# mvenouziou/Boosted_DETR

Hardware: AMD Instinct MI355X
Metric: images/sec training step (fwd+matcher+loss+bwd), 640x640 N=100 (higher is better)
Workload: dtype f32 (conv/GEMM products as 3 split-f16 [fwd] / split-bf16 [grad] MFMA products, f32 accumulate)

## Files before the change

boosted_detr_amd/_lib.py:

```python
from __future__ import annotations

import ctypes as C
import os
from pathlib import Path

_LIB_PATH = Path(os.environ.get("BDETR_LIB") or Path(__file__).resolve().parent / "csrc" / "libbdetr.so")
_lib = None

c_f32p = C.c_void_p
c_i32p = C.c_void_p
c_i64p = C.c_void_p
c_stream = C.c_void_p


class ConvDesc(C.Structure):
    _fields_ = [(n, C.c_int) for n in ("N", "H", "W", "C", "K", "R", "S", "stride", "pad", "OH", "OW")]


class GemmDesc(C.Structure):
    _fields_ = [
        ("I", C.c_int), ("J", C.c_int), ("R", C.c_int), ("nb0", C.c_int), ("nb1", C.c_int),
        ("a", C.c_void_p), ("lda", C.c_int64), ("sa0", C.c_int64), ("sa1", C.c_int64), ("a_rcontig", C.c_int),
        ("b", C.c_void_p), ("ldb", C.c_int64), ("sb0", C.c_int64), ("sb1", C.c_int64), ("b_rcontig", C.c_int),
        ("c", C.c_void_p), ("ldc", C.c_int64), ("sc0", C.c_int64), ("sc1", C.c_int64),
# ... 42 lines not shown
SIGNATURES = {
    "bdetr_abi_version": (I, []),
    "bdetr_last_error": (C.c_char_p, []),
    "bdetr_device_cus": (I, []),
    "bdetr_low_priority_stream_create": (I, [P]),
    "bdetr_side_stream_candidates": (I, [P, I, I, I, P, P, P]),
    "bdetr_stream_destroy": (I, [P]),
    "bdetr_stream_priority_range": (I, [P, P]),
    "bdetr_set_gemm_precision": (I, [I]),
    "bdetr_get_gemm_precision": (I, []),
    "bdetr_prof_enable": (I, [I]),
    "bdetr_prof_read": (I, [P, P, P]),
    "bdetr_prof_read_arith": (I, [I, P, P, P]),
    "bdetr_prof_dump": (I, [C.c_char_p]),
    "bdetr_image_prep": (I, [P, I, I, I, P, I, I, P]),
    "bdetr_tokens_prepare": (I, [P, P, L, I, I, I, P, P, P]),
    "bdetr_augment_ws_floats": (I, [I]),
    "bdetr_augment": (I, [P, P, P, P, I, I, I, P, P]),
    "bdetr_jpeg_quality_ws_bytes": (C.c_int64, [I, I, I]),
    "bdetr_jpeg_quality": (I, [P, P, P, I, I, I, P, P]),
    "bdetr_augment_jpeg": (I, [P, P, P, P, P, I, I, I, P, P, P]),
    "bdetr_conv2d_fwd": (I, [P, P, P, P, C.POINTER(ConvDesc), I, P, P, P]),
    "bdetr_conv2d_fwd_stat_chunks": (I, [C.POINTER(ConvDesc)]),
    "bdetr_conv2d_bwd_data": (I, [P, P, P, C.POINTER(ConvDesc), I, P]),
    "bdetr_conv2d_bwd_weight": (I, [P, P, P, C.POINTER(ConvDesc), I, P]),
    "bdetr_conv2d_bwd_weight_splitk": (I, [C.POINTER(ConvDesc)]),
    "bdetr_bn_apply_p16": (I, [P, P, P, P, P, P, I, C.POINTER(BnAffine), I, P, P, P, P, P, L, I, P]),
    "bdetr_bn_apply_p16_even_pixels": (I, [P, P, P, P, P, P, I, C.POINTER(BnAffine), I, P, P, P, P, P, L, I, I, I, P]),
    "bdetr_bn_bwd_p16": (I, [P, P, I, P, P, P, P, P, I, I, P, P, P, P, P, P, P, P, I, L, I, P]),
    "bdetr_bn_bwd_p16_even_pixels": (I, [P, P, I, P, P, P, P, P, I, I, P, P, P, P, P, P, I, I, I, I, I, P]),
# ... 32 lines not shown
    "bdetr_bn_stats_fold_rows": (I, []),
    "bdetr_bn_stats_frozen": (I, [P, P, I, F, P, P, P]),
    "bdetr_bn_apply": (I, [P, P, P, P, P, P, I, P, L, I, P]),
    "bdetr_bn_bwd_chunks": (I, [L]),
    "bdetr_bn_bwd": (I, [P, P, P, P, P, P, P, I, I, P, P, P, P, P, L, I, P]),
    "bdetr_bn_rows_stats": (I, [P, I, L, I, F, P, P, P, P, P]),
    "bdetr_bn_rows_apply": (I, [P, P, P, P, P, P, I, L, I, I, P, F, P, P, P, P]),
    "bdetr_bn_rows_bwd": (I, [P, P, P, P, P, I, I, P, P, P, P, I, L, I, P]),
    "bdetr_maxpool3x3s2_fwd": (I, [P, P, I, I, I, I, I, I, P]),
    "bdetr_maxpool3x3s2_bwd": (I, [P, P, P, P, I, I, I, I, I, I, P]),
    "bdetr_stem_pool_bwd_chunks": (I, [L]),
    "bdetr_stem_pool_fwd": (I, [P, P, P, P, P, I, I, I, I, P, P, P, P, P]),
    "bdetr_stem_pool_bwd": (I, [P, P, P, P, P, P, P, I, I, I, I, P, I, P, P, P, P]),
    "bdetr_p16_s2d_pack_bf16": (I, [P, I, I, I, P, P]),
    "bdetr_p16_stem_bwd_weight": (I, [P, P, P, I, I, I, I, P]),
    "bdetr_p16_s2d_unpack_dw": (I, [P, P, I, P]),
    "bdetr_attention_head_dim": (I, []),
    "bdetr_attention_fwd": (I, [P, P, P, P, P, I, I, I, I, F, P]),
    "bdetr_attention_bwd": (I, [P, P, P, P, P, P, P, P, P, P, I, I, I, I, F, P]),
    "bdetr_softmax_rows_fwd": (I, [P, P, L, I, F, P]),
    "bdetr_softmax_rows_bwd": (I, [P, P, P, L, I, F, P]),
    "bdetr_add_dropout_layernorm_fwd": (I, [P, P, P, P, P, P, P, L, I, F, F, U64, P, P]),
    "bdetr_ln_bwd_chunks": (I, [L]),
    "bdetr_add_dropout_layernorm_bwd": (I, [P, P, P, P, P, P, P, P, P, P, P, L, I, F, U64, P, I, P]),
    "bdetr_rowchain_fwd": (I, [C.POINTER(RowchainFwdDesc), P]),
    "bdetr_rowchain_bwd": (I, [C.POINTER(RowchainBwdDesc), P]),
    "bdetr_rowchain_reduce": (I, [P, I, C.POINTER(C.c_void_p * 7), C.POINTER(C.c_int * 7), P]),
    "bdetr_rowchain_width": (I, []),
    "bdetr_rowchain_pack_elems": (L, []),
    "bdetr_rowchain_partial_rows": (I, [L]),
# ... 88 lines not shown
```

boosted_detr_amd/backbone.py:

```python
from __future__ import annotations

from . import kernels as K
from . import ops
from .engine import Layer

RESNET50_STAGES = ((64, 3, 1), (128, 4, 2), (256, 6, 2), (512, 3, 2))
RESNET101_STAGES = ((64, 3, 1), (128, 4, 2), (256, 23, 2), (512, 3, 2))
RESNET_BN_EPS = 1.001e-5
KERAS_BN_EPS = 1e-3


class _ConvBN(Layer):

    def __init__(self, prefix: str, conv_name: str, bn_name: str, cin: int, cout: int, ksize: int, stride: int, pad: int,
                 pad_in_channels: int = 0, **kw):
        super().__init__(name=conv_name, scope_prefix=prefix, **kw)
        self.stride, self.pad = stride, pad
        self.kernel = self.add_weight("kernel", (ksize, ksize, cin, cout), "glorot_uniform", kind="conv_kernel",
                                      pad_in_channels=pad_in_channels)
        self.bias = self.add_weight("bias", (cout,), "zeros")
        self.name = bn_name
        gamma = self.add_weight("gamma", (cout,), "ones")
        beta = self.add_weight("beta", (cout,), "zeros")
        mm = self.add_weight("moving_mean", (cout,), "zeros", trainable=False)
# ... 66 lines not shown
        self.ImageFeaturesExtractor = ResNet(stages, name="resnet50" if model_name != "ResNet101" else "resnet101",
                                             scope_prefix=f"{self.scope}/", **kwargs)
        self.built = True

    def config(self):
        return self.get_config()

    def get_config(self):
        c = super().get_config()
        c.update({"image_input_shape": self.image_input_shape})
        return c

    def call(self, inputs, training=False):
        image = inputs[0]
        height, width = self.image_input_shape[:2]
        x = ops.image_prep(image, height, width)
        return self.ImageFeaturesExtractor([x], training=training)


class BackboneNeck(Layer):

    def __init__(self, encoder_dim, name="BackboneNeck", **kwargs):
        super().__init__(name=name, **kwargs)
        self.encoder_dim = encoder_dim

    def get_config(self):
        c = super().get_config()
        c.update({"encoder_dim": self.encoder_dim})
        return c

    def _bn(self, bn_name, c):
# ... 25 lines not shown
```

boosted_detr_amd/csrc/elementwise.hip:

```cpp
#include "common.h"

namespace {

__device__ __forceinline__ float prep_px(float v) {
    float q = floorf(v * 255.5f);
    return fminf(fmaxf(q, 0.f), 255.f);
}

__global__ __launch_bounds__(256) void image_prep_kernel(const float* __restrict__ in, int B, int h, int w,
                                                         float* __restrict__ out, int H, int W) {
    const int64_t npix = (int64_t)B * H * W;
    const float sy = (float)h / (float)H, sx = (float)w / (float)W;
    for (int64_t i = (int64_t)blockIdx.x * blockDim.x + threadIdx.x; i < npix; i += (int64_t)gridDim.x * blockDim.x) {
        const int ox = (int)(i % W); const int64_t t = i / W; const int oy = (int)(t % H); const int b = (int)(t / H);
        float rgb[3];
        if (h == H && w == W) {
            const float* p = in + i * 3;
#pragma unroll
            for (int c = 0; c < 3; ++c) rgb[c] = fminf(fmaxf(p[c], 0.f), 1.f);
        } else {
            const float fy = ((float)oy + 0.5f) * sy - 0.5f, fx = ((float)ox + 0.5f) * sx - 0.5f;
            const float fy0 = floorf(fy), fx0 = floorf(fx);
            const int y0 = max((int)fy0, 0), y1 = min((int)ceilf(fy), h - 1);
            const int x0 = max((int)fx0, 0), x1 = min((int)ceilf(fx), w - 1);
            const float ly = fy - fy0, lx = fx - fx0;
            const float* base = in + (int64_t)b * h * w * 3;
#pragma unroll
            for (int c = 0; c < 3; ++c) {
                auto px = [&](int yy, int xx) { return fminf(fmaxf(base[((int64_t)yy * w + xx) * 3 + c], 0.f), 1.f); };
                const float top = px(y0, x0) + (px(y0, x1) - px(y0, x0)) * lx;
                const float bot = px(y1, x0) + (px(y1, x1) - px(y1, x0)) * lx;
                rgb[c] = top + (bot - top) * ly;
            }
        }
        f32x4 o;
        o[0] = prep_px(rgb[2]) - 103.939f;
        o[1] = prep_px(rgb[1]) - 116.779f;
        o[2] = prep_px(rgb[0]) - 123.68f;
        o[3] = 0.f;
        reinterpret_cast<f32x4*>(out)[i] = o;
    }
}

__global__ __launch_bounds__(256) void maxpool_fwd_kernel(const float* __restrict__ x, float* __restrict__ y,
                                                          int N, int H, int W, int C, int OH, int OW) {
    const int c4n = C / 4;
    const int64_t n4 = (int64_t)N * OH * OW * c4n;
    for (int64_t i = (int64_t)blockIdx.x * blockDim.x + threadIdx.x; i < n4; i += (int64_t)gridDim.x * blockDim.x) {
        const int c4 = (int)(i % c4n); int64_t t = i / c4n;
        const int ow = (int)(t % OW); t /= OW; const int oh = (int)(t % OH); const int n = (int)(t / OH);
        f32x4 m = {-INFINITY, -INFINITY, -INFINITY, -INFINITY};
#pragma unroll
        for (int r = 0; r < 3; ++r)
#pragma unroll
            for (int s = 0; s < 3; ++s) {
// ... 191 lines not shown
                       reinterpret_cast<unsigned long long*>(log), cursor, cap, (unsigned long long)tag);
    return bdetr_launch_status("debug_checksum");
}

extern "C" int bdetr_flag_nonfinite(const float* x, int64_t n, int* flag, void* stream) {
    BDETR_CHECK_ARG(x && flag && n > 0, "bdetr_flag_nonfinite: bad arguments");
    hipLaunchKernelGGL(flag_nonfinite_kernel, dim3(ew_grid(n, 256, 4)), dim3(256), 0, (hipStream_t)stream, x, n, flag);
    return bdetr_launch_status("flag_nonfinite");
}

extern "C" int bdetr_image_prep(const float* in, int B, int h, int w, float* out, int H, int W, void* stream) {
    BDETR_CHECK_ARG(in && out && B > 0 && h > 0 && w > 0 && H > 0 && W > 0, "bdetr_image_prep: bad arguments");
    int64_t n = (int64_t)B * H * W;
    hipLaunchKernelGGL(image_prep_kernel, dim3(ew_grid(n, 256, 1)), dim3(256), 0, (hipStream_t)stream, in, B, h, w, out, H, W);
    return bdetr_launch_status("image_prep");
}

extern "C" int bdetr_maxpool3x3s2_fwd(const float* x, float* y, int N, int H, int W, int C, int OH, int OW, void* stream) {
    BDETR_CHECK_ARG(x && y && C % 4 == 0 && OH == (H + 2 - 3) / 2 + 1 && OW == (W + 2 - 3) / 2 + 1, "bdetr_maxpool3x3s2_fwd: bad arguments");
    int64_t n4 = (int64_t)N * OH * OW * (C / 4);
    hipLaunchKernelGGL(maxpool_fwd_kernel, dim3(ew_grid(n4, 256, 1)), dim3(256), 0, (hipStream_t)stream, x, y, N, H, W, C, OH, OW);
    return bdetr_launch_status("maxpool_fwd");
}
extern "C" int bdetr_maxpool3x3s2_bwd(const float* x, const float* y, const float* dy, float* dx,
                                      int N, int H, int W, int C, int OH, int OW, void* stream) {
    BDETR_CHECK_ARG(x && y && dy && dx && C % 4 == 0 && OH == (H + 2 - 3) / 2 + 1 && OW == (W + 2 - 3) / 2 + 1, "bdetr_maxpool3x3s2_bwd: bad arguments");
    int64_t n4 = (int64_t)N * H * W * (C / 4);
    hipLaunchKernelGGL(maxpool_bwd_kernel, dim3(ew_grid(n4, 256, 1)), dim3(256), 0, (hipStream_t)stream, x, y, dy, dx, N, H, W, C, OH, OW);
    return bdetr_launch_status("maxpool_bwd");
}
// ... 165 lines not shown
```

boosted_detr_amd/csrc/p16.hip:

```cpp
#include "p16.h"

namespace {

__global__ __launch_bounds__(256) void p16_pack_kernel(const float* __restrict__ x, int64_t n8, void* __restrict__ f16_out, void* __restrict__ bf16_out,
                                                       int* __restrict__ overflow_flag, float f16_scale) {
    for (int64_t i = (int64_t)blockIdx.x * blockDim.x + threadIdx.x; i < n8; i += (int64_t)gridDim.x * blockDim.x) {
        const f32x4 a = reinterpret_cast<const f32x4*>(x)[2 * i], b = reinterpret_cast<const f32x4*>(x)[2 * i + 1];
        const float v[8] = {a[0], a[1], a[2], a[3], b[0], b[1], b[2], b[3]};
        if (f16_out) {
            const float vs[8] = {v[0] * f16_scale, v[1] * f16_scale, v[2] * f16_scale, v[3] * f16_scale, v[4] * f16_scale, v[5] * f16_scale, v[6] * f16_scale, v[7] * f16_scale};
            p16_store8<true>(reinterpret_cast<char*>(f16_out) + i * 32, vs);
            if (overflow_flag && p16_f16_overflow(vs)) *overflow_flag = 1;
        }
        if (bf16_out) p16_store8<false>(reinterpret_cast<char*>(bf16_out) + i * 32, v);
    }
}

template <bool F16>
__global__ __launch_bounds__(256) void p16_unpack_kernel(const void* __restrict__ p, int64_t n8, float* __restrict__ out) {
    for (int64_t i = (int64_t)blockIdx.x * blockDim.x + threadIdx.x; i < n8; i += (int64_t)gridDim.x * blockDim.x) {
        float v[8];
        p16_load8<F16>(reinterpret_cast<const char*>(p) + i * 32, v);
        reinterpret_cast<f32x4*>(out)[2 * i] = f32x4{v[0], v[1], v[2], v[3]};
        reinterpret_cast<f32x4*>(out)[2 * i + 1] = f32x4{v[4], v[5], v[6], v[7]};
// ... 30 lines not shown
            if (overflow_flag && p16_f16_overflow(v)) *overflow_flag = 1;
        }
        if (wt != nullptr) {
            const int c = (int)(i % C); int64_t t = i / C;
            const int tap = (int)(t % (R * S)); const int kg = (int)(t / (R * S));
            const int r = tap / S, s2 = tap - r * S;
            const int src_tap = (R - 1 - r) * S + (S - 1 - s2);
            float v[8];
#pragma unroll
            for (int e = 0; e < 8; ++e) v[e] = w[((int64_t)(kg * 8 + e) * R * S + src_tap) * C + c];
            p16_store8<false>(wt + (((int64_t)c * R * S + tap) * K + kg * 8) * 4, v);
        }
    }
}

}

extern "C" int bdetr_p16_pack_conv_weights_multi(const int64_t* table, int ntensors, int* overflow_flag, void* stream) {
    BDETR_CHECK_ARG(table && ntensors > 0, "bdetr_p16_pack_conv_weights_multi: bad arguments");
    hipLaunchKernelGGL(p16_pack_weights_multi_kernel, dim3(48, ntensors), dim3(256), 0, (hipStream_t)stream, table, overflow_flag);
    return bdetr_launch_status("p16_pack_conv_weights_multi");
}

extern "C" int bdetr_p16_pack(const float* x, int64_t n, void* f16_out, void* bf16_out, int* overflow_flag, void* stream) {
    BDETR_CHECK_ARG(x && n > 0 && n % 8 == 0 && (f16_out || bf16_out), "bdetr_p16_pack: bad arguments (n %% 8 == 0 required)");
    hipLaunchKernelGGL(p16_pack_kernel, dim3(ew_grid(n / 8, 256, 2)), dim3(256), 0, (hipStream_t)stream, x, n / 8, f16_out, bf16_out, overflow_flag, 1.f);
    return bdetr_launch_status("p16_pack");
}

extern "C" int bdetr_p16_unpack(const void* p, int is_f16, int64_t n, float* out, void* stream) {
    BDETR_CHECK_ARG(p && out && n > 0 && n % 8 == 0, "bdetr_p16_unpack: bad arguments (n %% 8 == 0 required)");
    if (is_f16) hipLaunchKernelGGL((p16_unpack_kernel<true>), dim3(ew_grid(n / 8, 256, 2)), dim3(256), 0, (hipStream_t)stream, p, n / 8, out);
    else        hipLaunchKernelGGL((p16_unpack_kernel<false>), dim3(ew_grid(n / 8, 256, 2)), dim3(256), 0, (hipStream_t)stream, p, n / 8, out);
    return bdetr_launch_status("p16_unpack");
}
// ... 46 lines not shown
```

boosted_detr_amd/csrc/sgemm.hip:

```cpp
#include "gemm_common.h"
#include "p16.h"
#include <stdlib.h>
#include <string.h>
#include <type_traits>
#include <utility>

using namespace bdgemm;

namespace {

constexpr int BK = 32;
constexpr unsigned OOB = 0xFFFFFFF0u;
constexpr unsigned NUM_RECORDS = 0xFFFFFF00u;

typedef __bf16 bf16x8 __attribute__((ext_vector_type(8)));
typedef _Float16 f16x8 __attribute__((ext_vector_type(8)));
typedef unsigned int u32x4 __attribute__((ext_vector_type(4)));
typedef unsigned int u32x2 __attribute__((ext_vector_type(2)));
typedef short s16x4 __attribute__((ext_vector_type(4)));
typedef __attribute__((address_space(3))) void lds_void;

__device__ __forceinline__ __amdgpu_buffer_rsrc_t make_rsrc(const void* p, unsigned records = NUM_RECORDS) {
    const unsigned long long a = reinterpret_cast<unsigned long long>(p);
    const unsigned lo = __builtin_amdgcn_readfirstlane((unsigned)a), hi = __builtin_amdgcn_readfirstlane((unsigned)(a >> 32));
// ... 958 lines not shown
    return splitk_fold(ws, zdim, slab, dw, n, st);
}
extern "C" int bdetr_p16_conv2d_bwd_weight_ws(const void* x, int x_is_f16, const void* dy_bf16, float* dw,
                                              const bdetr_conv_desc* d, int splitk, float* ws, int64_t ws_elems, void* stream) {
    return p16_bwd_weight(x, x_is_f16, dy_bf16, dw, d, splitk, stream, ws, ws_elems);
}
extern "C" int bdetr_p16_conv2d_bwd_weight(const void* x_bf16, const void* dy_bf16, float* dw,
                                           const bdetr_conv_desc* d, int splitk, void* stream) {
    return p16_bwd_weight(x_bf16, 0, dy_bf16, dw, d, splitk, stream);
}
extern "C" int bdetr_p16_conv2d_bwd_weight_xf16(const void* x_f16, const void* dy_bf16, float* dw,
                                                const bdetr_conv_desc* d, int splitk, void* stream) {
    return p16_bwd_weight(x_f16, 1, dy_bf16, dw, d, splitk, stream);
}

extern "C" int bdetr_p16_stem_bwd_weight(const void* x2_bf16, const void* dy_bf16, float* dw2, int N, int H2, int W2, int K, void* stream) {
    BDETR_CHECK_ARG(x2_bf16 && dy_bf16 && dw2 && N > 0 && H2 > 0 && W2 > 0 && K > 0 && K % 64 == 0 && aligned16(x2_bf16) && aligned16(dy_bf16),
                    "bdetr_p16_stem_bwd_weight: bad arguments (K %% 64 == 0)");
    const int64_t M64 = (int64_t)N * H2 * W2;
    BDETR_CHECK_ARG(M64 < (1LL << 31) && span_ok(M64 * 16) && span_ok(M64 * K), "bdetr_p16_stem_bwd_weight: tensors of 4 GB or more");
    const int M = (int)M64, Kd = 4 * 4 * 16;
    GemmParams g; init_params(g);
    g.I = K; g.J = Kd; g.R = M; g.c = dw2; g.ldc = Kd;
    const int64_t tiles = cdiv64(K, 64) * cdiv64(Kd, 64);
    int64_t sk = (16LL * num_cus()) / tiles;
    const int64_t maxsk = cdiv64(M, 8LL * BK);
    if (sk > maxsk) sk = maxsk;
    if (sk < 1) sk = 1;
    if (sk > 1024) sk = 1024;
    int zdim = 1;
    if (sk > 1) {
        g.r_chunk = (int)(cdiv64(cdiv64(M, sk), BK) * BK);
        zdim = (int)cdiv64(M, g.r_chunk);
        g.splitk = zdim > 1 ? zdim : 2;
        g.mode = ST_ATOMIC;
    }
    PDense a{dy_bf16, (unsigned)K, M, K};
    PPatch b = make_patch(x2_bf16, N, H2, W2, 16, H2, W2, 4, 4, 1, 2, M, Kd);
    return launch_any<XXDense, XXPatch, true, false>(a, b, g, zdim, (hipStream_t)stream, 3000, T_64x64);
}
```

boosted_detr_amd/kernels.py:

```python
from __future__ import annotations

import ctypes as C
from dataclasses import dataclass
from typing import Optional, Tuple

import numpy as np
import torch

from . import _lib
from ._lib import BnAffine, BnBwdFuse, ConvDesc, GemmDesc, LossDesc, RowchainBwdDesc, RowchainFwdDesc, check

ACT_NONE, ACT_RELU, ACT_TANH = 0, 1, 2


_LAUNCH_STREAM = [None]


def set_launch_stream(handle: Optional[int]) -> Optional[int]:
    prev = _LAUNCH_STREAM[0]
    _LAUNCH_STREAM[0] = handle
    return prev


GEMM_FP32, GEMM_BF16X3, GEMM_MIXED, GEMM_SPLIT, GEMM_BF16X6 = 0, 1, 2, 3, 4
# ... 77 lines not shown
        if not t.is_contiguous():
            raise _lib.BdetrError("kernel operands must be contiguous")


def empty(*shape, like: torch.Tensor, dtype=torch.float32) -> torch.Tensor:
    return torch.empty(shape, dtype=dtype, device=like.device)


def image_prep(image: torch.Tensor, H: int, W: int) -> torch.Tensor:
    _chk(image)
    B, h, w, c = image.shape
    assert c == 3
    out = empty(B, H, W, 4, like=image)
    check(_lib.lib().bdetr_image_prep(_p(image), B, h, w, _p(out), H, W, _stream()), "image_prep")
    return out


def tokens_prepare(cat_ids: torch.Tensor, att_ids: torch.Tensor, C_: int, A: int):
    _chk(cat_ids, att_ids, dtype=torch.int32)
    if cat_ids.dim() == 3:
        cat_ids = cat_ids[..., 0].contiguous()
    B, M = cat_ids.shape
    slots = att_ids.shape[2] if att_ids.dim() == 3 else 1
    cat = torch.empty_like(cat_ids)
    hot = torch.empty((B, M, A), dtype=torch.float32, device=cat_ids.device)
    check(_lib.lib().bdetr_tokens_prepare(_p(cat_ids), _p(att_ids), B * M, slots, C_, A, _p(cat), _p(hot), _stream()), "tokens_prepare")
    return cat, hot


def augment(image: torch.Tensor, iparams: torch.Tensor, fparams: torch.Tensor, quality: Optional[torch.Tensor] = None) -> torch.Tensor:
# ... 554 lines not shown

def stem_pool_bwd(dpool, tap, y, mean, rstd, gamma, beta, dgamma=None, dbeta=None, dy_p16=False):
    _chk(dpool, y, mean, rstd, gamma, beta, dgamma, dbeta)
    assert tap.is_cuda and tap.is_contiguous() and tap.dtype == torch.uint8 and tuple(tap.shape) == tuple(dpool.shape)
    L = _lib.lib()
    N, H, W, Cc = y.shape
    dy = torch.empty_like(y)
    dgamma = empty(Cc, like=y) if dgamma is None else dgamma
    dbeta = empty(Cc, like=y) if dbeta is None else dbeta
    ws = empty(2 * Cc * L.bdetr_stem_pool_bwd_chunks(N * H * W), like=y)
    check(L.bdetr_stem_pool_bwd(_p(dpool), _p(tap), _p(y), _p(mean), _p(rstd), _p(gamma), _p(beta), N, H, W, Cc, _p(dy), int(dy_p16), _p(dgamma), _p(dbeta),
                                _p(ws), _stream()), "stem_pool_bwd")
    return dy, dgamma, dbeta


def stem_bwd_weight_s2d(x4, dy_bf16, dw):
    _chk(x4, dy_bf16, dw)
    L = _lib.lib()
    N, H, W, Cc = x4.shape
    Kout = dw.shape[0]
    assert Cc == 4 and H % 2 == 0 and W % 2 == 0 and tuple(dw.shape) == (Kout, 7, 7, 4) and tuple(dy_bf16.shape) == (N, H // 2, W // 2, Kout)
    x2 = empty(N, H // 2, W // 2, 16, like=x4)
    check(L.bdetr_p16_s2d_pack_bf16(_p(x4), N, H, W, _p(x2), _stream()), "p16_s2d_pack_bf16")
    dw2 = empty(Kout, 4, 4, 16, like=x4)
    check(L.bdetr_zero(_p(dw2), dw2.numel(), _stream()), "zero")
    check(L.bdetr_p16_stem_bwd_weight(_p(x2), _p(dy_bf16), _p(dw2), N, H // 2, W // 2, Kout, _stream()), "p16_stem_bwd_weight")
    check(L.bdetr_p16_s2d_unpack_dw(_p(dw2), _p(dw), Kout, _stream()), "p16_s2d_unpack_dw")
    return dw


def attention_fwd(q, k, v, heads, scale):
    _chk(q, k, v)
    B, nq, D = q.shape
    nk = k.shape[1]
    o = empty(B, heads, nq, D // heads, like=q)
    lse = empty(B, heads, nq, like=q)
    check(_lib.lib().bdetr_attention_fwd(_p(q), _p(k), _p(v), _p(o), _p(lse), B, heads, nq, nk, scale, _stream()), "attention_fwd")
    return o, lse


def attention_bwd(q, k, v, o, d_o, lse, heads, scale):
# ... 809 lines not shown
```

boosted_detr_amd/ops.py:

```python
from __future__ import annotations

import math
import os
import weakref
from typing import Optional

import numpy as np
import torch

from . import kernels as K
from . import _lib
from .engine import WEIGHTS_VERSION, Variable, capture, current_tape, dense_contribution, info, materialise, own, side_task, tag

_dropout_site = [0]
_dropout_seed_dev = [None]


def dropout_seed_tensor() -> torch.Tensor:
    if _dropout_seed_dev[0] is None:
        _dropout_seed_dev[0] = torch.full((1,), 0x5EED, dtype=torch.int64, device="cuda")
    return _dropout_seed_dev[0]


def set_dropout_seed(seed: int, write: bool = True) -> None:
# ... 476 lines not shown
        g, mine = g.contiguous(), info(g).owned
        return tuple(own(g[l * B:(l + 1) * B]) if mine else g[l * B:(l + 1) * B] for l in range(L))

    _rec([out], list(xs), backward)
    return out


def maxpool(x: torch.Tensor) -> torch.Tensor:
    y = K.maxpool_fwd(x)
    _rec([y], [x], lambda g: (own(K.maxpool_bwd(x, y, g.contiguous())),))
    return y


STEM_FUSE = os.environ.get("BDETR_STEM_FUSE", "1") != "0"
STEM_S2D = os.environ.get("BDETR_STEM_S2D", "1") != "0"


def conv_bn_relu_maxpool(x: torch.Tensor, w: Variable, b: Variable, bn: BNState, stride: int, pad: int, training: bool,
                         bn_batch_stats: bool) -> torch.Tensor:
    N, H, W, Cin = x.shape
    Kout, R, S, _ = w.value.shape
    if not (STEM_FUSE and training and bn_batch_stats and _p16_active() and Kout % 8 == 0):
        return maxpool(conv_bn(x, w, b, bn, stride, pad, True, training=training, bn_batch_stats=bn_batch_stats, x_needs_grad=False))
    g = K.ConvGeom(N, H, W, Cin, Kout, R, S, stride, pad)
    x32 = as_fp32(x)
    y, parts = K.conv2d_fwd(x32, w.value, b.value, g, K.ACT_NONE, want_stats=True)
    if parts is None or parts[0] is None:
        parts = K.colstats(_2d(y))
    mean, rstd = K.bn_stats(g.M, Kout, parts, bn.eps, bn.momentum, True, bn.moving_mean.value, bn.moving_var.value, like=y)
    _, out, tap = K.stem_pool_fwd(y, mean, rstd, bn.gamma.value, bn.beta.value)
    attach_packed(out, out.detach(), p16_only=True)

    def backward(g_out):
        sg, sb = GradSink(bn.gamma), GradSink(bn.beta)
        s2d = (STEM_S2D and w.needs_grad and (R, S, stride, pad, Cin) == (7, 7, 2, 3, 4) and H % 2 == 0 and W % 2 == 0 and Kout % 64 == 0
               and K.get_gemm_precision() in ("split", "mixed") and not K.deterministic())
        dy, _, _ = K.stem_pool_bwd(materialise(g_out).contiguous(), tap, y, mean, rstd, bn.gamma.value, bn.beta.value, dgamma=sg.buf, dbeta=sb.buf,
                                   dy_p16=s2d)
        sg.commit()
        sb.commit()
        if s2d:
            _param_grads_task(w, b, lambda dw, pz: K.stem_bwd_weight_s2d(x32, dy, dw), None, x32, dy)
        else:
            _param_grads_task(w, b, lambda dw, pz: K.conv2d_bwd_weight(x32, dy, g, dw=dw, prezeroed=pz), None, x32, dy)
        return (None,)

    _rec([out], [x], backward)
    return out


def dense(x: torch.Tensor, w: Variable, b: Variable, act: int = K.ACT_NONE) -> torch.Tensor:
    x2d = _2d(x)
    y2d = K.linear_fwd(x2d, w.value, b.value, act)
    y = y2d.view(*x.shape[:-1], w.value.shape[0])

    def backward(g_out, acc=None):
        g2d = _2d(g_out.contiguous())
# ... 279 lines not shown
```

boosted_detr_amd/training.py:

```python
from __future__ import annotations

import contextlib
import glob
import math
import os
import sys
import time
from dataclasses import dataclass
from typing import Dict, Iterable, List, NamedTuple, Optional

import numpy as np
import torch

from . import _lib
from . import engine
from . import kernels as K
from . import ops
from .inference import Inference
from .engine import Layer, Tape, Variable, bump_weights_version, device, join_side_stream, recording, to_device


class CosineDecayRestarts:

    def __init__(self, initial_learning_rate, first_decay_steps, t_mul=2.0, m_mul=1.0, alpha=0.0):
# ... 914 lines not shown
        entry = self._graphs.get(sig)
        if entry is None:
            n = self._graph_warm.get(sig, 0)
            self._graph_warm[sig] = n + 1
            if n < 2 or getattr(self.optimizer, "flat_grad", None) is None:
                return None
            static = {k: v.clone() for k, v in data.items()}
            ops.set_dropout_seed(self._step_seed())
            self.optimizer.stage_lr()
            keep = (self.steps_done, self.optimizer.iterations)
            if self._dp is not None:
                self._dp.drain()
            cap = engine.SegmentedCapture()
            engine.set_capture(cap)
            prev_launch = K.set_launch_stream(None)
            try:
                cap.begin_main()
                logs = self._device_step(static, stage_scalars=False)
                cap.end_main()
                cap.sides.append(None)
            except BaseException:
                cap.abort()
                self.steps_done, self.optimizer.iterations = keep
                raise
            finally:
                engine.set_capture(None)
                K.set_launch_stream(prev_launch)
            cap.done = []
            if cap.CENSUS:
                self._graph_census = cap.census()
            self.steps_done, self.optimizer.iterations = keep
            entry = (cap, static, logs, (list(self._step_losses), list(self._loss_roots), dict(self._step_metrics)))
            self._graphs[sig] = entry
        cap, static, logs, book = entry
        for k, v in data.items():
            if v is not static[k]:
                static[k].copy_(v)
        ops.set_dropout_seed(self._step_seed())
        self.optimizer.stage_lr()
        cap.replay(engine.side_stream() if os.environ.get("BDETR_GRAPH_SIDE", "1") != "0" else None)
# ... 152 lines not shown
```

include/bdetr.h:

```cpp
#ifndef BDETR_H
#define BDETR_H
#include <stdint.h>
#ifdef __cplusplus
extern "C" {
#endif

#define BDETR_ABI_VERSION 8

int         bdetr_abi_version(void);
const char* bdetr_last_error(void);
int         bdetr_device_cus(void);

int         bdetr_low_priority_stream_create(void** stream_out);
int         bdetr_stream_priority_range(int* least, int* greatest);
int         bdetr_side_stream_candidates(void* main_stream, int ncand, int loads, int ticks, void** streams_out, float* scores_ms, float* unloaded_ms);
int         bdetr_stream_destroy(void* stream);

enum { BDETR_GEMM_FP32 = 0, BDETR_GEMM_BF16X3 = 1, BDETR_GEMM_MIXED = 2, BDETR_GEMM_SPLIT = 3, BDETR_GEMM_BF16X6 = 4 };
int         bdetr_set_gemm_precision(int mode);
int         bdetr_get_gemm_precision(void);

int bdetr_prof_enable(int on);
int bdetr_prof_read(double* total_ms, int64_t* launches, double* flops);
int bdetr_prof_read_arith(int arith, double* total_ms, int64_t* launches, double* flops);
int bdetr_prof_dump(const char* path);

enum { BDETR_ACT_NONE = 0, BDETR_ACT_RELU = 1, BDETR_ACT_TANH = 2 };

int bdetr_image_prep(const float* in, int B, int h, int w, float* out, int H, int W, void* stream);

int bdetr_tokens_prepare(const int* cat_ids, const int* att_ids, int64_t rows, int slots, int C, int A,
                         int* cat_out, float* att_hot, void* stream);

int bdetr_augment_ws_floats(int B);
int bdetr_augment(const float* in, float* out, const int32_t* iparams, const float* fparams,
                  int B, int H, int W, float* ws, void* stream);
int64_t bdetr_jpeg_quality_ws_bytes(int B, int H, int W);
int bdetr_jpeg_quality(const float* in, float* out, const int32_t* quality, int B, int H, int W, void* ws, void* stream);
int bdetr_augment_jpeg(const float* in, float* out, const int32_t* iparams, const float* fparams, const int32_t* quality,
                       int B, int H, int W, float* ws, void* jpeg_ws, void* stream);

typedef struct {
    int N, H, W, C;
    int K, R, S;
// ... 111 lines not shown
int bdetr_bn_rows_bwd(const float* dout, const float* x, const float* mean, const float* rstd, const float* gamma,
                      int grouped_stats, int frozen, float* dx, float* dgamma, float* dbeta, float* ws, int G, int64_t R, int C,
                      void* stream);

int bdetr_maxpool3x3s2_fwd(const float* x, float* y, int N, int H, int W, int C, int OH, int OW, void* stream);
int bdetr_maxpool3x3s2_bwd(const float* x, const float* y, const float* dy, float* dx,
                           int N, int H, int W, int C, int OH, int OW, void* stream);

int bdetr_stem_pool_bwd_chunks(int64_t rows);
int bdetr_stem_pool_fwd(const float* y, const float* mean, const float* rstd, const float* gamma, const float* beta,
                        int N, int H, int W, int C, float* out32, void* out_f16, uint8_t* tap, int* overflow_flag, void* stream);
int bdetr_stem_pool_bwd(const float* dpool, const uint8_t* tap, const float* y, const float* mean, const float* rstd, const float* gamma,
                        const float* beta, int N, int H, int W, int C, float* dy, int dy_p16 , float* dgamma, float* dbeta, float* ws, void* stream);
int bdetr_p16_s2d_pack_bf16(const float* x, int N, int H, int W, void* out_bf16, void* stream);
int bdetr_p16_stem_bwd_weight(const void* x2_bf16, const void* dy_bf16, float* dw2, int N, int H2, int W2, int K, void* stream);
int bdetr_p16_s2d_unpack_dw(const float* dw2, float* dw, int K, void* stream);

int bdetr_softmax_rows_fwd(const float* s, float* p, int64_t rows, int cols, float scale, void* stream);
int bdetr_softmax_rows_bwd(const float* p, const float* dp, float* ds, int64_t rows, int cols, float scale, void* stream);

int bdetr_attention_head_dim(void);
int bdetr_attention_fwd(const float* q, const float* k, const float* v, float* o, float* lse,
                        int B, int h, int nq, int nk, float scale, void* stream);
int bdetr_attention_bwd(const float* q, const float* k, const float* v, const float* o, const float* d_o,
                        const float* lse, float* dq, float* dk, float* dv, float* dvec_ws,
                        int B, int h, int nq, int nk, float scale, void* stream);

int bdetr_add_dropout_layernorm_fwd(const float* x, const float* y, const float* gamma, const float* beta,
                                    float* out, float* mean, float* rstd, int64_t rows, int D,
                                    float eps, float rate, uint64_t seed, const uint64_t* seed_base, void* stream);
// ... 168 lines not shown
```

Baseline: 658.0.

## Fuse stem s2d packing into image prep, widen stem dW tile, tile weight packing

Image preprocessing now also writes the space-to-depth bf16 copy used by the stem weight-gradient GEMM, which removes a separate pack pass over the input. The dW2 buffer is zeroed during the forward pass instead of in backward. The stem bwd-weight GEMM uses a wider 64x256 tile with less split-K. A new tiled, LDS-transposed multi-tensor conv weight packing kernel replaces the old one, and Python GC is disabled during graph capture. The changes are mostly independent and add env switches plus extra code paths.

```diff
diff --git a/boosted_detr_amd/_lib.py b/boosted_detr_amd/_lib.py
--- a/boosted_detr_amd/_lib.py
+++ b/boosted_detr_amd/_lib.py
@@ -80,6 +80,7 @@
     "bdetr_prof_read_arith": (I, [I, P, P, P]),
     "bdetr_prof_dump": (I, [C.c_char_p]),
     "bdetr_image_prep": (I, [P, I, I, I, P, I, I, P]),
+    "bdetr_image_prep_s2d": (I, [P, I, I, I, P, I, I, P, P]),
     "bdetr_tokens_prepare": (I, [P, P, L, I, I, I, P, P, P]),
     "bdetr_augment_ws_floats": (I, [I]),
     "bdetr_augment": (I, [P, P, P, P, I, I, I, P, P]),
@@ -142,6 +143,7 @@
     "bdetr_stem_pool_bwd": (I, [P, P, P, P, P, P, P, I, I, I, I, P, I, P, P, P, P]),
     "bdetr_p16_s2d_pack_bf16": (I, [P, I, I, I, P, P]),
     "bdetr_p16_stem_bwd_weight": (I, [P, P, P, I, I, I, I, P]),
+    "bdetr_p16_stem_bwd_weight_splitk": (I, [P, P, P, I, I, I, I, I, P]),
     "bdetr_p16_s2d_unpack_dw": (I, [P, P, I, P]),
     "bdetr_attention_head_dim": (I, []),
     "bdetr_attention_fwd": (I, [P, P, P, P, P, I, I, I, I, F, P]),
diff --git a/boosted_detr_amd/backbone.py b/boosted_detr_amd/backbone.py
--- a/boosted_detr_amd/backbone.py
+++ b/boosted_detr_amd/backbone.py
@@ -104,7 +104,8 @@
     def call(self, inputs, training=False):
         image = inputs[0]
         height, width = self.image_input_shape[:2]
-        x = ops.image_prep(image, height, width)
+        st = self.ImageFeaturesExtractor.stem
+        x = ops.image_prep_for_stem(image, height, width, st.kernel, st.stride, st.pad, training, training and st.trainable)
         return self.ImageFeaturesExtractor([x], training=training)
 
 
diff --git a/boosted_detr_amd/csrc/elementwise.hip b/boosted_detr_amd/csrc/elementwise.hip
--- a/boosted_detr_amd/csrc/elementwise.hip
+++ b/boosted_detr_amd/csrc/elementwise.hip
@@ -1,10 +1,39 @@
-#include "common.h"
+#include "p16.h"
 
 namespace {
 
 __device__ __forceinline__ float prep_px(float v) {
     float q = floorf(v * 255.5f);
     return fminf(fmaxf(q, 0.f), 255.f);
+}
+
+__device__ __forceinline__ f32x4 image_prep_pixel(const float* __restrict__ in, int h, int w, int H, int W, float sy, float sx, int64_t i, int b, int oy, int ox) {
+    float rgb[3];
+    if (h == H && w == W) {
+        const float* p = in + i * 3;
+#pragma unroll
+        for (int c = 0; c < 3; ++c) rgb[c] = fminf(fmaxf(p[c], 0.f), 1.f);
+    } else {
+        const float fy = ((float)oy + 0.5f) * sy - 0.5f, fx = ((float)ox + 0.5f) * sx - 0.5f;
+        const float fy0 = floorf(fy), fx0 = floorf(fx);
+        const int y0 = max((int)fy0, 0), y1 = min((int)ceilf(fy), h - 1);
+        const int x0 = max((int)fx0, 0), x1 = min((int)ceilf(fx), w - 1);
+        const float ly = fy - fy0, lx = fx - fx0;
+        const float* base = in + (int64_t)b * h * w * 3;
+#pragma unroll
+        for (int c = 0; c < 3; ++c) {
+            auto px = [&](int yy, int xx) { return fminf(fmaxf(base[((int64_t)yy * w + xx) * 3 + c], 0.f), 1.f); };
+            const float top = px(y0, x0) + (px(y0, x1) - px(y0, x0)) * lx;
+            const float bot = px(y1, x0) + (px(y1, x1) - px(y1, x0)) * lx;
+            rgb[c] = top + (bot - top) * ly;
+        }
+    }
+    f32x4 o;
+    o[0] = prep_px(rgb[2]) - 103.939f;
+    o[1] = prep_px(rgb[1]) - 116.779f;
+    o[2] = prep_px(rgb[0]) - 123.68f;
+    o[3] = 0.f;
+    return o;
 }
 
 __global__ __launch_bounds__(256) void image_prep_kernel(const float* __restrict__ in, int B, int h, int w,
@@ -13,32 +42,23 @@
     const float sy = (float)h / (float)H, sx = (float)w / (float)W;
     for (int64_t i = (int64_t)blockIdx.x * blockDim.x + threadIdx.x; i < npix; i += (int64_t)gridDim.x * blockDim.x) {
         const int ox = (int)(i % W); const int64_t t = i / W; const int oy = (int)(t % H); const int b = (int)(t / H);
-        float rgb[3];
-        if (h == H && w == W) {
-            const float* p = in + i * 3;
-#pragma unroll
-            for (int c = 0; c < 3; ++c) rgb[c] = fminf(fmaxf(p[c], 0.f), 1.f);
-        } else {
-            const float fy = ((float)oy + 0.5f) * sy - 0.5f, fx = ((float)ox + 0.5f) * sx - 0.5f;
-            const float fy0 = floorf(fy), fx0 = floorf(fx);
-            const int y0 = max((int)fy0, 0), y1 = min((int)ceilf(fy), h - 1);
-            const int x0 = max((int)fx0, 0), x1 = min((int)ceilf(fx), w - 1);
-            const float ly = fy - fy0, lx = fx - fx0;
-            const float* base = in + (int64_t)b * h * w * 3;
-#pragma unroll
-            for (int c = 0; c < 3; ++c) {
-                auto px = [&](int yy, int xx) { return fminf(fmaxf(base[((int64_t)yy * w + xx) * 3 + c], 0.f), 1.f); };
-                const float top = px(y0, x0) + (px(y0, x1) - px(y0, x0)) * lx;
-                const float bot = px(y1, x0) + (px(y1, x1) - px(y1, x0)) * lx;
-                rgb[c] = top + (bot - top) * ly;
-            }
-        }
-        f32x4 o;
-        o[0] = prep_px(rgb[2]) - 103.939f;
-        o[1] = prep_px(rgb[1]) - 116.779f;
-        o[2] = prep_px(rgb[0]) - 123.68f;
-        o[3] = 0.f;
-        reinterpret_cast<f32x4*>(out)[i] = o;
+        reinterpret_cast<f32x4*>(out)[i] = image_prep_pixel(in, h, w, H, W, sy, sx, i, b, oy, ox);
+    }
+}
+
+__global__ __launch_bounds__(256) void image_prep_s2d_kernel(const float* __restrict__ in, int B, int h, int w,
+                                                             float* __restrict__ out, int H, int W, void* __restrict__ x2) {
+    const int H2 = H >> 1, W2 = W >> 1;
+    const int64_t n = (int64_t)B * H * W;
+    const float sy = (float)h / (float)H, sx = (float)w / (float)W;
+    for (int64_t u = (int64_t)blockIdx.x * blockDim.x + threadIdx.x; u < n; u += (int64_t)gridDim.x * blockDim.x) {
+        const int ab = (int)(u & 3); const int64_t t = u >> 2;
+        const int j = (int)(t % W2); const int64_t q = t / W2; const int i2 = (int)(q % H2); const int b = (int)(q / H2);
+        const int oy = 2 * i2 + (ab >> 1), ox = 2 * j + (ab & 1);
+        const int64_t i = ((int64_t)b * H + oy) * W + ox;
+        const f32x4 p = image_prep_pixel(in, h, w, H, W, sy, sx, i, b, oy, ox);
+        reinterpret_cast<f32x4*>(out)[i] = p;
+        p16_store4<false>(x2, u, p[0], p[1], p[2], p[3]);
     }
 }
 
@@ -260,6 +280,12 @@
     int64_t n = (int64_t)B * H * W;
     hipLaunchKernelGGL(image_prep_kernel, dim3(ew_grid(n, 256, 1)), dim3(256), 0, (hipStream_t)stream, in, B, h, w, out, H, W);
     return bdetr_launch_status("image_prep");
+}
+extern "C" int bdetr_image_prep_s2d(const float* in, int B, int h, int w, float* out, int H, int W, void* x2_bf16, void* stream) {
+    BDETR_CHECK_ARG(in && out && x2_bf16 && B > 0 && h > 0 && w > 0 && H > 0 && W > 0 && H % 2 == 0 && W % 2 == 0, "bdetr_image_prep_s2d: bad arguments (even H and W)");
+    int64_t n = (int64_t)B * H * W;
+    hipLaunchKernelGGL(image_prep_s2d_kernel, dim3(ew_grid(n, 256, 1)), dim3(256), 0, (hipStream_t)stream, in, B, h, w, out, H, W, x2_bf16);
+    return bdetr_launch_status("image_prep_s2d");
 }
 
 extern "C" int bdetr_maxpool3x3s2_fwd(const float* x, float* y, int N, int H, int W, int C, int OH, int OW, void* stream) {
diff --git a/boosted_detr_amd/csrc/p16.hip b/boosted_detr_amd/csrc/p16.hip
--- a/boosted_detr_amd/csrc/p16.hip
+++ b/boosted_detr_amd/csrc/p16.hip
@@ -1,4 +1,6 @@
 #include "p16.h"
+#include <stdlib.h>
+#include <string.h>
 
 namespace {
 
@@ -68,11 +70,93 @@
     }
 }
 
+constexpr int PACK_T = 64, PACK_LD = PACK_T + 1;
+constexpr int PACK_ROWS = 256;
+__global__ __launch_bounds__(256) void p16_pack_weights_tiled_kernel(const int64_t* __restrict__ table, int ntensors, int* __restrict__ overflow_flag) {
+    __shared__ float tile[PACK_T * PACK_LD];
+    __shared__ int last[PACK_ROWS];
+    const int tid = threadIdx.x;
+    {
+        int n = 0;
+        if (tid < ntensors) {
+            const int64_t* row = table + (int64_t)tid * 7;
+            if (row[1] != 0 || row[2] != 0) n = (int)(row[4] * row[5] * ((row[3] + PACK_T - 1) / PACK_T) * ((row[6] + PACK_T - 1) / PACK_T));
+        }
+        last[tid] = n;
+        __syncthreads();
+        for (int d = 1; d < PACK_ROWS; d <<= 1) {
+            const int v = tid >= d ? last[tid - d] : 0;
+            __syncthreads();
+            last[tid] += v;
+            __syncthreads();
+        }
+    }
+    const int total = last[PACK_ROWS - 1];
+    for (int item = blockIdx.x; item < total; item += gridDim.x) {
+        int t = 0;
+        for (int hi = ntensors - 1; t < hi;) { const int mid = (t + hi) >> 1; if (last[mid] > item) hi = mid; else t = mid + 1; }
+        const int64_t* row = table + (int64_t)t * 7;
+        const float* w = reinterpret_cast<const float*>(row[0]);
+        char* wf = reinterpret_cast<char*>(row[1]);
+        char* wt = reinterpret_cast<char*>(row[2]);
+        const int K = (int)row[3], T = (int)(row[4] * row[5]), C = (int)row[6];
+        const int ctiles = (C + PACK_T - 1) / PACK_T;
+        int q = item - (t > 0 ? last[t - 1] : 0);
+        const int c0 = (q % ctiles) * PACK_T; q /= ctiles;
+        const int src_tap = q % T, k0 = (q / T) * PACK_T;
+        const int g8 = tid & 7, r32 = tid >> 3;
+#pragma unroll
+        for (int pass = 0; pass < PACK_T / 32; ++pass) {
+            const int kl = pass * 32 + r32, k = k0 + kl, c = c0 + g8 * 8;
+            if (k < K && c < C) {
+                const int64_t at = ((int64_t)k * T + src_tap) * C + c;
+                const f32x4 a = *reinterpret_cast<const f32x4*>(w + at), b = *reinterpret_cast<const f32x4*>(w + at + 4);
+                if (wf != nullptr) {
+                    const float v[8] = {a[0] * P16_W_SCALE, a[1] * P16_W_SCALE, a[2] * P16_W_SCALE, a[3] * P16_W_SCALE,
+                                        b[0] * P16_W_SCALE, b[1] * P16_W_SCALE, b[2] * P16_W_SCALE, b[3] * P16_W_SCALE};
+                    p16_store8<true>(wf + at * 4, v);
+                    if (overflow_flag && p16_f16_overflow(v)) *overflow_flag = 1;
+                }
+                if (wt != nullptr) {
+                    float* d = tile + kl * PACK_LD + g8 * 8;
+                    d[0] = a[0]; d[1] = a[1]; d[2] = a[2]; d[3] = a[3]; d[4] = b[0]; d[5] = b[1]; d[6] = b[2]; d[7] = b[3];
+                }
+            }
+        }
+        if (wt != nullptr) {
+            __syncthreads();
+            const int tap = T - 1 - src_tap;
+#pragma unroll
+            for (int pass = 0; pass < PACK_T / 32; ++pass) {
+                const int cl = pass * 32 + r32, c = c0 + cl, k = k0 + g8 * 8;
+                if (c < C && k < K) {
+                    float v[8];
+#pragma unroll
+                    for (int e = 0; e < 8; ++e) v[e] = tile[(g8 * 8 + e) * PACK_LD + cl];
+                    p16_store8<false>(wt + (((int64_t)c * T + tap) * K + k) * 4, v);
+                }
+            }
+            __syncthreads();
+        }
+    }
+}
+
+bool pack_tiled() {
+    const char* e = getenv("BDETR_PACK_TILED");
+    return !(e && !strcmp(e, "0"));
+}
+
 }
 
 extern "C" int bdetr_p16_pack_conv_weights_multi(const int64_t* table, int ntensors, int* overflow_flag, void* stream) {
     BDETR_CHECK_ARG(table && ntensors > 0, "bdetr_p16_pack_conv_weights_multi: bad arguments");
-    hipLaunchKernelGGL(p16_pack_weights_multi_kernel, dim3(48, ntensors), dim3(256), 0, (hipStream_t)stream, table, overflow_flag);
+    if (pack_tiled()) {
+        for (int first = 0; first < ntensors; first += PACK_ROWS)
+            hipLaunchKernelGGL(p16_pack_weights_tiled_kernel, dim3(2048), dim3(256), 0, (hipStream_t)stream, table + (int64_t)first * 7,
+                               ntensors - first < PACK_ROWS ? ntensors - first : PACK_ROWS, overflow_flag);
+    } else {
+        hipLaunchKernelGGL(p16_pack_weights_multi_kernel, dim3(48, ntensors), dim3(256), 0, (hipStream_t)stream, table, overflow_flag);
+    }
     return bdetr_launch_status("p16_pack_conv_weights_multi");
 }
 
diff --git a/boosted_detr_amd/csrc/sgemm.hip b/boosted_detr_amd/csrc/sgemm.hip
--- a/boosted_detr_amd/csrc/sgemm.hip
+++ b/boosted_detr_amd/csrc/sgemm.hip
@@ -996,18 +996,23 @@
     return p16_bwd_weight(x_f16, 1, dy_bf16, dw, d, splitk, stream);
 }
 
-extern "C" int bdetr_p16_stem_bwd_weight(const void* x2_bf16, const void* dy_bf16, float* dw2, int N, int H2, int W2, int K, void* stream) {
+static int stem_wide_tile() {
+    const char* e = getenv("BDETR_STEM_DW_WIDE");
+    return (e && !strcmp(e, "0")) ? 0 : 1;
+}
+extern "C" int bdetr_p16_stem_bwd_weight_splitk(const void* x2_bf16, const void* dy_bf16, float* dw2, int N, int H2, int W2, int K, int splitk, void* stream) {
     BDETR_CHECK_ARG(x2_bf16 && dy_bf16 && dw2 && N > 0 && H2 > 0 && W2 > 0 && K > 0 && K % 64 == 0 && aligned16(x2_bf16) && aligned16(dy_bf16),
                     "bdetr_p16_stem_bwd_weight: bad arguments (K %% 64 == 0)");
     const int64_t M64 = (int64_t)N * H2 * W2;
     BDETR_CHECK_ARG(M64 < (1LL << 31) && span_ok(M64 * 16) && span_ok(M64 * K), "bdetr_p16_stem_bwd_weight: tensors of 4 GB or more");
     const int M = (int)M64, Kd = 4 * 4 * 16;
+    const bool wide = stem_wide_tile() != 0;
     GemmParams g; init_params(g);
     g.I = K; g.J = Kd; g.R = M; g.c = dw2; g.ldc = Kd;
-    const int64_t tiles = cdiv64(K, 64) * cdiv64(Kd, 64);
-    int64_t sk = (16LL * num_cus()) / tiles;
+    const int64_t tiles = cdiv64(K, 64) * cdiv64(Kd, wide ? 256 : 64);
+    int64_t sk = splitk > 0 ? splitk : ((wide ? 2LL : 16LL) * num_cus()) / tiles;
     const int64_t maxsk = cdiv64(M, 8LL * BK);
-    if (sk > maxsk) sk = maxsk;
+    if (splitk <= 0 && sk > maxsk) sk = maxsk;
     if (sk < 1) sk = 1;
     if (sk > 1024) sk = 1024;
     int zdim = 1;
@@ -1019,5 +1024,9 @@
     }
     PDense a{dy_bf16, (unsigned)K, M, K};
     PPatch b = make_patch(x2_bf16, N, H2, W2, 16, H2, W2, 4, 4, 1, 2, M, Kd);
+    if (wide) return launch_cfg<64, 256, 2, 4, 2, XXDense, XXPatch, true, false, false, 4>(a, b, g, zdim, (hipStream_t)stream, 3000);
     return launch_any<XXDense, XXPatch, true, false>(a, b, g, zdim, (hipStream_t)stream, 3000, T_64x64);
 }
+extern "C" int bdetr_p16_stem_bwd_weight(const void* x2_bf16, const void* dy_bf16, float* dw2, int N, int H2, int W2, int K, void* stream) {
+    return bdetr_p16_stem_bwd_weight_splitk(x2_bf16, dy_bf16, dw2, N, H2, W2, K, 0, stream);
+}
diff --git a/boosted_detr_amd/kernels.py b/boosted_detr_amd/kernels.py
--- a/boosted_detr_amd/kernels.py
+++ b/boosted_detr_amd/kernels.py
@@ -115,6 +115,22 @@
     out = empty(B, H, W, 4, like=image)
     check(_lib.lib().bdetr_image_prep(_p(image), B, h, w, _p(out), H, W, _stream()), "image_prep")
     return out
+
+
+def image_prep_s2d(image: torch.Tensor, H: int, W: int):
+    _chk(image)
+    B, h, w, c = image.shape
+    assert c == 3 and H % 2 == 0 and W % 2 == 0
+    out = empty(B, H, W, 4, like=image)
+    x2 = empty(B, H // 2, W // 2, 16, like=image)
+    check(_lib.lib().bdetr_image_prep_s2d(_p(image), B, h, w, _p(out), H, W, _p(x2), _stream()), "image_prep_s2d")
+    return out, x2
+
+
+def stem_dw2_zeros(Kout: int, like: torch.Tensor) -> torch.Tensor:
+    dw2 = empty(Kout, 4, 4, 16, like=like)
+    check(_lib.lib().bdetr_zero(_p(dw2), dw2.numel(), _stream()), "zero")
+    return dw2
 
 
 def tokens_prepare(cat_ids: torch.Tensor, att_ids: torch.Tensor, C_: int, A: int):
@@ -699,17 +715,19 @@
     return dy, dgamma, dbeta
 
 
-def stem_bwd_weight_s2d(x4, dy_bf16, dw):
-    _chk(x4, dy_bf16, dw)
+def stem_bwd_weight_s2d(x4, dy_bf16, dw, splitk: int = 0, x2=None, dw2=None):
+    _chk(x4, dy_bf16, dw, x2, dw2)
     L = _lib.lib()
     N, H, W, Cc = x4.shape
     Kout = dw.shape[0]
     assert Cc == 4 and H % 2 == 0 and W % 2 == 0 and tuple(dw.shape) == (Kout, 7, 7, 4) and tuple(dy_bf16.shape) == (N, H // 2, W // 2, Kout)
-    x2 = empty(N, H // 2, W // 2, 16, like=x4)
-    check(L.bdetr_p16_s2d_pack_bf16(_p(x4), N, H, W, _p(x2), _stream()), "p16_s2d_pack_bf16")
-    dw2 = empty(Kout, 4, 4, 16, like=x4)
-    check(L.bdetr_zero(_p(dw2), dw2.numel(), _stream()), "zero")
-    check(L.bdetr_p16_stem_bwd_weight(_p(x2), _p(dy_bf16), _p(dw2), N, H // 2, W // 2, Kout, _stream()), "p16_stem_bwd_weight")
+    if x2 is None:
+        x2 = empty(N, H // 2, W // 2, 16, like=x4)
+        check(L.bdetr_p16_s2d_pack_bf16(_p(x4), N, H, W, _p(x2), _stream()), "p16_s2d_pack_bf16")
+    if dw2 is None:
+        dw2 = stem_dw2_zeros(Kout, x4)
+    assert tuple(x2.shape) == (N, H // 2, W // 2, 16) and tuple(dw2.shape) == (Kout, 4, 4, 16)
+    check(L.bdetr_p16_stem_bwd_weight_splitk(_p(x2), _p(dy_bf16), _p(dw2), N, H // 2, W // 2, Kout, int(splitk), _stream()), "p16_stem_bwd_weight")
     check(L.bdetr_p16_s2d_unpack_dw(_p(dw2), _p(dw), Kout, _stream()), "p16_s2d_unpack_dw")
     return dw
 
diff --git a/boosted_detr_amd/ops.py b/boosted_detr_amd/ops.py
--- a/boosted_detr_amd/ops.py
+++ b/boosted_detr_amd/ops.py
@@ -514,13 +514,35 @@
 
 STEM_FUSE = os.environ.get("BDETR_STEM_FUSE", "1") != "0"
 STEM_S2D = os.environ.get("BDETR_STEM_S2D", "1") != "0"
+STEM_S2D_PREP = os.environ.get("BDETR_STEM_S2D_PREP", "1") != "0"
+
+
+def _stem_s2d(x_shape, w: Variable, stride: int, pad: int) -> bool:
+    _, H, W, Cin = x_shape
+    Kout, R, S, _ = w.value.shape
+    return (STEM_S2D and w.needs_grad and (R, S, stride, pad, Cin) == (7, 7, 2, 3, 4) and H % 2 == 0 and W % 2 == 0 and Kout % 64 == 0
+            and K.get_gemm_precision() in ("split", "mixed") and not K.deterministic())
+
+
+def _stem_fused(w: Variable, training: bool, bn_batch_stats: bool) -> bool:
+    return bool(STEM_FUSE and training and bn_batch_stats and _p16_active() and w.value.shape[0] % 8 == 0)
+
+
+def image_prep_for_stem(image: torch.Tensor, H: int, W: int, w: Optional[Variable], stride: int, pad: int, training: bool,
+                        bn_batch_stats: bool) -> torch.Tensor:
+    if (STEM_S2D_PREP and w is not None and current_tape() is not None and _stem_fused(w, training, bn_batch_stats)
+            and _stem_s2d((image.shape[0], H, W, 4), w, stride, pad)):
+        x, x2 = K.image_prep_s2d(image, H, W)
+        x._stem_x2 = x2
+        return x
+    return K.image_prep(image, H, W)
 
 
 def conv_bn_relu_maxpool(x: torch.Tensor, w: Variable, b: Variable, bn: BNState, stride: int, pad: int, training: bool,
                          bn_batch_stats: bool) -> torch.Tensor:
     N, H, W, Cin = x.shape
     Kout, R, S, _ = w.value.shape
-    if not (STEM_FUSE and training and bn_batch_stats and _p16_active() and Kout % 8 == 0):
+    if not _stem_fused(w, training, bn_batch_stats):
         return maxpool(conv_bn(x, w, b, bn, stride, pad, True, training=training, bn_batch_stats=bn_batch_stats, x_needs_grad=False))
     g = K.ConvGeom(N, H, W, Cin, Kout, R, S, stride, pad)
     x32 = as_fp32(x)
@@ -530,17 +552,19 @@
     mean, rstd = K.bn_stats(g.M, Kout, parts, bn.eps, bn.momentum, True, bn.moving_mean.value, bn.moving_var.value, like=y)
     _, out, tap = K.stem_pool_fwd(y, mean, rstd, bn.gamma.value, bn.beta.value)
     attach_packed(out, out.detach(), p16_only=True)
+    x2 = getattr(x, "_stem_x2", None) if _stem_s2d(x.shape, w, stride, pad) else None
+    zeroed = [K.stem_dw2_zeros(Kout, x32) if x2 is not None else None]
 
     def backward(g_out):
         sg, sb = GradSink(bn.gamma), GradSink(bn.beta)
-        s2d = (STEM_S2D and w.needs_grad and (R, S, stride, pad, Cin) == (7, 7, 2, 3, 4) and H % 2 == 0 and W % 2 == 0 and Kout % 64 == 0
-               and K.get_gemm_precision() in ("split", "mixed") and not K.deterministic())
+        s2d = _stem_s2d(x.shape, w, stride, pad)
         dy, _, _ = K.stem_pool_bwd(materialise(g_out).contiguous(), tap, y, mean, rstd, bn.gamma.value, bn.beta.value, dgamma=sg.buf, dbeta=sb.buf,
                                    dy_p16=s2d)
         sg.commit()
         sb.commit()
         if s2d:
-            _param_grads_task(w, b, lambda dw, pz: K.stem_bwd_weight_s2d(x32, dy, dw), None, x32, dy)
+            dw2, zeroed[0] = zeroed[0], None
+            _param_grads_task(w, b, lambda dw, pz: K.stem_bwd_weight_s2d(x32, dy, dw, x2=x2, dw2=dw2), None, x32, dy, x2, dw2)
         else:
             _param_grads_task(w, b, lambda dw, pz: K.conv2d_bwd_weight(x32, dy, g, dw=dw, prezeroed=pz), None, x32, dy)
         return (None,)
diff --git a/boosted_detr_amd/training.py b/boosted_detr_amd/training.py
--- a/boosted_detr_amd/training.py
+++ b/boosted_detr_amd/training.py
@@ -1,6 +1,7 @@
 from __future__ import annotations
 
 import contextlib
+import gc
 import glob
 import math
 import os
@@ -952,6 +953,9 @@
             cap = engine.SegmentedCapture()
             engine.set_capture(cap)
             prev_launch = K.set_launch_stream(None)
+            gc.collect()
+            gc_was_on = gc.isenabled()
+            gc.disable()
             try:
                 cap.begin_main()
                 logs = self._device_step(static, stage_scalars=False)
@@ -962,6 +966,8 @@
                 self.steps_done, self.optimizer.iterations = keep
                 raise
             finally:
+                if gc_was_on:
+                    gc.enable()
                 engine.set_capture(None)
                 K.set_launch_stream(prev_launch)
             cap.done = []
diff --git a/include/bdetr.h b/include/bdetr.h
--- a/include/bdetr.h
+++ b/include/bdetr.h
@@ -28,6 +28,7 @@
 enum { BDETR_ACT_NONE = 0, BDETR_ACT_RELU = 1, BDETR_ACT_TANH = 2 };
 
 int bdetr_image_prep(const float* in, int B, int h, int w, float* out, int H, int W, void* stream);
+int bdetr_image_prep_s2d(const float* in, int B, int h, int w, float* out, int H, int W, void* x2_bf16, void* stream);
 
 int bdetr_tokens_prepare(const int* cat_ids, const int* att_ids, int64_t rows, int slots, int C, int A,
                          int* cat_out, float* att_hot, void* stream);
@@ -169,6 +170,7 @@
                         const float* beta, int N, int H, int W, int C, float* dy, int dy_p16 , float* dgamma, float* dbeta, float* ws, void* stream);
 int bdetr_p16_s2d_pack_bf16(const float* x, int N, int H, int W, void* out_bf16, void* stream);
 int bdetr_p16_stem_bwd_weight(const void* x2_bf16, const void* dy_bf16, float* dw2, int N, int H2, int W2, int K, void* stream);
+int bdetr_p16_stem_bwd_weight_splitk(const void* x2_bf16, const void* dy_bf16, float* dw2, int N, int H2, int W2, int K, int splitk, void* stream);
 int bdetr_p16_s2d_unpack_dw(const float* dw2, float* dw, int K, void* stream);
 
 int bdetr_softmax_rows_fwd(const float* s, float* p, int64_t rows, int cols, float scale, void* stream);
```

Result: no change. 661.3, median of 5 (+0.5%).
